# astra-vision/SceneRF

Hardware: NVIDIA H100
Metric: rays/sec (higher is better)
Workload: dtype fp32 (2 x fp16 split operands, fp32 accumulate)

## Files before the change

scenerf_b200/csrc/mlp_tc.cu:

```cuda
#include <cuda.h>
#include <cuda_fp16.h>
#include <cstdio>
#include <cstdlib>
#include <cstring>
#include <type_traits>
#include "kernels.cuh"
#include "tma.cuh"

namespace srf {
namespace tc {

constexpr int kTileM = 64;
constexpr int kChunkK = 64;
constexpr int kAChunkBytes = kTileM * 128;
constexpr int kBRows = 128, kBSlotBytes = kBRows * 128;
constexpr int kHiddenChunks = kHidden / kChunkK;
constexpr int kQuarters = kHidden / kBRows;
constexpr int kOutN = 16;
constexpr int kOutImgBytes = kOutN * 128;
constexpr int kThreads = 256;
constexpr int kNumBias = 8;
constexpr size_t kHeaderBytes = (size_t)kNumBias * kHidden * sizeof(float);
constexpr int kNumLayers = 11;
constexpr int kScaleSlot = 7 * kHidden + 256, kInvScaleSlot = 7 * kHidden + 257;
constexpr size_t kScratchFloats = (size_t)2 * kTileM * kHidden;
constexpr size_t kExchangeOffset = (size_t)2 * 2 * 64 * 128;

constexpr int kSmemAct = 0;
constexpr int kSmemX = kSmemAct + kHiddenChunks * kAChunkBytes;
constexpr int kSmemZ = kSmemX + kAChunkBytes;
constexpr int kRingBytes = 4 * kBSlotBytes;
constexpr int kSmemRing = kSmemZ + 2 * kAChunkBytes;
constexpr int kSmemBar = kSmemRing + 2 * kRingBytes;
constexpr int kSmemSph = kSmemBar + 2 * 4 * 8;
constexpr int kSmemMask = kSmemSph + kTileM * 4;
constexpr int kSmemTotal = kSmemMask + 16;
static_assert(kSmemTotal + 1024 <= 232448, "shared memory budget");

struct Layer { int chunks_is_kz, chunks, fresh, signal, is_out; };
__constant__ Layer kLayers[kNumLayers] = {
    {0, 1, 1, 0, 0}, {1, 0, 0, 1, 0},
    {0, 8, 1, 1, 0}, {0, 8, 1, 0, 0}, {1, 0, 0, 1, 0},
    {0, 8, 1, 1, 0}, {0, 8, 1, 0, 0}, {1, 0, 0, 1, 0},
    {0, 8, 1, 1, 0}, {0, 8, 1, 1, 0},
    {0, 8, 1, 1, 1}};

struct KernelArgs {
  const float* pts;
  const float* viewdir;
  int n, n_per, n_tiles, kz;
  const unsigned char* wblob;
  float* scratch;
  float* raw_out;
  int d_out;
  int32_t* dbg_sphere;
  int skip_zero;
  int hidden_fp16;
  const unsigned char* preproj;
  int pre_W1, pre_H1;
  int debug_layer;
  float* debug_acc;
  int* error_flag;
};

__device__ __forceinline__ void fence_proxy_async_smem() { asm volatile("fence.proxy.async.shared::cta;" ::: "memory"); }

__device__ __forceinline__ uint64_t l2_policy_evict_last() {
  uint64_t pol;
  asm volatile("createpolicy.fractional.L2::evict_last.b64 %0, 1.0;" : "=l"(pol));
  return pol;
}
__device__ __forceinline__ void bulk_g2s(uint32_t dst_smem, const void* src, uint32_t bytes, uint32_t bar, uint64_t policy) {
  asm volatile("cp.async.bulk.shared::cluster.global.mbarrier::complete_tx::bytes.L2::cache_hint [%0], [%1], %2, [%3], %4;"
               ::"r"(dst_smem), "l"(src), "r"(bytes), "r"(bar), "l"(policy)
               : "memory");
}
__device__ __forceinline__ void named_bar_sync(int id, int threads) {
  asm volatile("bar.sync %0, %1;" ::"r"(id), "r"(threads) : "memory");
}
__device__ __forceinline__ void sts128(uint32_t addr, uint32_t a, uint32_t b, uint32_t c, uint32_t d) {
  asm volatile("st.shared.v4.b32 [%0], {%1, %2, %3, %4};" ::"r"(addr), "r"(a), "r"(b), "r"(c), "r"(d) : "memory");
}
__device__ __forceinline__ void sts32(uint32_t addr, uint32_t a) {
  asm volatile("st.shared.b32 [%0], %1;" ::"r"(addr), "r"(a) : "memory");
}
__device__ __forceinline__ uint32_t pack_relu_half2(float lo, float hi) {
  uint32_t d;
  asm("cvt.rn.relu.f16x2.f32 %0, %1, %2;" : "=r"(d) : "f"(hi), "f"(lo));
  return d;
}
__device__ __forceinline__ uint32_t pack_half2(float lo, float hi) {
  __half2 h = __floats2half2_rn(lo, hi);
  return *reinterpret_cast<uint32_t*>(&h);
}
__device__ __forceinline__ void split_half2(float a, float b, uint32_t& hi, uint32_t& lo) {
  const __half2 h = __floats2half2_rn(a, b);
  const float2 hf = __half22float2(h);
  const __half2 l = __floats2half2_rn(a - hf.x, b - hf.y);
  hi = *reinterpret_cast<const uint32_t*>(&h);
  lo = *reinterpret_cast<const uint32_t*>(&l);
}

__device__ __forceinline__ uint32_t sw128_offset(int row, int g) { return (uint32_t)(row * 128 + ((g ^ (row & 7)) << 4)); }

__device__ __forceinline__ int layer_chunks(int l, int kz) { return kLayers[l].chunks_is_kz ? kz : kLayers[l].chunks; }
__device__ __forceinline__ bool chunk_active(int l, int c, uint64_t mask) { return !kLayers[l].chunks_is_kz || ((mask >> c) & 1ull); }

__device__ __forceinline__ uint64_t chunk_mask_for_scales(const DevParams& p, uint32_t scale_bits, int kz) {
  uint64_t m = 0;
  for (int c = 0; c < kz; ++c) {
    const int lo = c * kChunkK, hi = lo + kChunkK;
    for (int s = 0; s < kScales; ++s)
      if (((scale_bits >> s) & 1u) && p.ch_off[s] < hi && p.ch_off[s + 1] > lo) m |= 1ull << c;
  }
  return m;
}

__device__ __forceinline__ size_t chunk_image_offset(int l, int k, int kz, int parts) {
  size_t off = 0;
  for (int i = 0; i < l; ++i) off += (size_t)layer_chunks(i, kz) * (kLayers[i].is_out ? kOutImgBytes : kQuarters * kBSlotBytes);
  return (off + (size_t)k * (kLayers[l].is_out ? kOutImgBytes : kQuarters * kBSlotBytes)) * (size_t)parts;
}

struct Cursor {
  int l = 0, k = 0, j = 0;
  __device__ __forceinline__ bool normalize(int kz, uint64_t mask, int last_layer, int wg) {
    while (l <= last_layer) {
      if (l == kNumLayers - 1 && wg != 0) return false;
      if (j >= (kLayers[l].is_out ? 1 : 2)) { j = 0; ++k; }
      if (k >= layer_chunks(l, kz)) { k = 0; ++l; continue; }
      if (!chunk_active(l, k, mask)) { ++k; continue; }
      return true;
    }
    return false;
  }
};

__device__ __forceinline__ int next_active(int kz, uint64_t mask, int c) {
  for (++c; c < kz; ++c)
    if ((mask >> c) & 1ull) return c;
  return -1;
}

template <bool H16, bool SPLIT, bool PRE>
__global__ void __launch_bounds__(kThreads, 1)
point_mlp_tc_kernel(const __grid_constant__ DevParams p, const __grid_constant__ KernelArgs a) {
  extern __shared__ __align__(1024) unsigned char smem_dyn[];
  unsigned char* smem = smem_dyn + ((1024u - (smem_u32(smem_dyn) & 1023u)) & 1023u);
  const uint32_t smem_base = smem_u32(smem);
  const int tid = threadIdx.x;
  const int wg = tid >> 7, t = tid & 127, w = t >> 5, lane = tid & 31;
  constexpr int kParts = SPLIT ? 2 : 1;
  constexpr int kPts = SPLIT ? kTileM / 2 : kTileM;
  constexpr int kSlotBytes = kBSlotBytes * kParts;
  constexpr int kSlots = kRingBytes / kSlotBytes;
  const uint32_t ring = smem_base + kSmemRing + (uint32_t)wg * kRingBytes;
  auto full_bar = [&](int s) { return smem_base + kSmemBar + 8u * (uint32_t)(wg * 4 + s); };
  short2* sph_smem = reinterpret_cast<short2*>(smem + kSmemSph);
  volatile unsigned long long* mask_smem = reinterpret_cast<volatile unsigned long long*>(smem + kSmemMask);

  if (tid == 0) {
    for (int s = 0; s < 8; ++s) mbar_init(smem_base + kSmemBar + 8u * s, 1);
    fence_barrier_init();
  }
  __syncthreads();

  const int kz = a.kz;
  const int last_layer = (a.debug_layer >= 0) ? a.debug_layer : (kNumLayers - 1);
  const unsigned char* images = a.wblob + kHeaderBytes;
  const float* bias = reinterpret_cast<const float*>(a.wblob);
  float* scratch = a.scratch + (size_t)blockIdx.x * kScratchFloats;
  float* hbuf = scratch + (size_t)wg * (2 * 64 * 128);
  float* xbuf = scratch + kExchangeOffset + (size_t)wg * (2 * 64 * 64);
  const uint64_t policy = l2_policy_evict_last();

  Cursor pc;
  bool p_live = false;
  uint32_t ppos = 0, cpos = 0, done = 0;
  uint64_t mask = 0;
  auto produce = [&]() {
    if (t != 0) return;
    while (p_live && ppos < done + (uint32_t)kSlots) {
      const bool is_out = kLayers[pc.l].is_out != 0;
      const unsigned char* src = images + chunk_image_offset(pc.l, pc.k, kz, kParts) + (is_out ? 0 : (size_t)(2 * wg + pc.j) * kSlotBytes);
      const uint32_t bytes = is_out ? (uint32_t)(kOutImgBytes * kParts) : (uint32_t)kSlotBytes;
      const int s = (int)(ppos % kSlots);
      mbar_arrive_expect_tx(full_bar(s), bytes);
      bulk_g2s(ring + (uint32_t)s * kSlotBytes, src, bytes, full_bar(s), policy);
      ++ppos;
      ++pc.j;
      p_live = pc.normalize(kz, mask, last_layer, wg);
    }
  };
  float acc0[64], acc1[64], acco[8];
  auto wait_slot = [&]() -> uint32_t {
    const int s = (int)(cpos % kSlots);
    mbar_wait<kWatchPointMlp>(full_bar(s), (cpos / kSlots) & 1u, a.error_flag);
    return ring + (uint32_t)s * kSlotBytes;
  };
  auto release1 = [&]() {
    gmma::wait<1>();
    done = cpos - 1;
    produce();
  };
  auto mma_pair = [&](uint32_t a_addr, bool fresh) {
    const uint64_t ad = gmma::desc_sw128(a_addr);
    {
      const uint32_t b = wait_slot();
      gmma::fence();
#pragma unroll
      for (int k = 0; k < 4; ++k)
#pragma unroll
        for (int part = 0; part < kParts; ++part)
          gmma::mma_f16_n128(acc0, ad + 2 * k, gmma::desc_sw128(b + part * kBSlotBytes) + 2 * k, (fresh && k == 0 && part == 0) ? 0 : 1);
      gmma::commit();
      ++cpos;
    }
    release1();
    {
      const uint32_t b = wait_slot();
      gmma::fence();
#pragma unroll
      for (int k = 0; k < 4; ++k)
#pragma unroll
        for (int part = 0; part < kParts; ++part)
          gmma::mma_f16_n128(acc1, ad + 2 * k, gmma::desc_sw128(b + part * kBSlotBytes) + 2 * k, (fresh && k == 0 && part == 0) ? 0 : 1);
      gmma::commit();
      ++cpos;
    }
  };
  auto mma_out = [&](uint32_t a_addr, bool fresh) {
    const uint64_t ad = gmma::desc_sw128(a_addr);
    const uint32_t b = wait_slot();
    gmma::fence();
#pragma unroll
    for (int k = 0; k < 4; ++k)
#pragma unroll
      for (int part = 0; part < kParts; ++part)
        gmma::mma_f16_n16(acco, ad + 2 * k, gmma::desc_sw128(b + part * kOutImgBytes) + 2 * k, (fresh && k == 0 && part == 0) ? 0 : 1);
    gmma::commit();
    ++cpos;
  };
  auto retire1 = release1;
  auto retire0 = [&]() {
    gmma::wait<0>();
    gmma::fence_regs(acc0); gmma::fence_regs(acc1); gmma::fence_regs(acco);
    done = cpos;
    produce();
  };
  auto sync_all = [&]() { named_bar_sync(1, kThreads); };

  const short2* sph_cur = sph_smem;
  const int erow0 = 16 * w + (lane >> 2);
  const int ecol = 2 * (lane & 3);

  for (int tile = blockIdx.x; tile < a.n_tiles; tile += gridDim.x) {
    const int row0 = tile * kPts;
    if (tid == 0) mask_smem[0] = 0ull;
    sync_all();
    {
      uint32_t my_scales = 0;
      if (tid < kPts) {
        const int gi = row0 + tid;
        int sx = kSphereInvalid, sy = kSphereInvalid;
        if (gi < a.n) {
          point_to_sphere(p, a.pts[(size_t)gi * 3 + 0], a.pts[(size_t)gi * 3 + 1], a.pts[(size_t)gi * 3 + 2], sx, sy);
          if (a.dbg_sphere) { a.dbg_sphere[(size_t)gi * 2 + 0] = sx; a.dbg_sphere[(size_t)gi * 2 + 1] = sy; }
        }
        sph_smem[tid] = make_short2((short)max(min(sx, 32767), -32768), (short)max(min(sy, 32767), -32768));
        if (a.skip_zero) {
#pragma unroll
          for (int s = 0; s < kScales; ++s) my_scales |= scale_taps(p, s, sx, sy).any ? (1u << s) : 0u;
        }
      }
      if (a.skip_zero && tid < ((kPts + 31) & ~31)) {
        const uint32_t wbits = __reduce_or_sync(0xffffffffu, my_scales);
        if (lane == 0) {
          const unsigned long long bits = chunk_mask_for_scales(p, wbits, kz);
          if (bits) atomicOr((unsigned long long*)mask_smem, bits);
        }
      }
    }
    sync_all();
    mask = PRE ? 0ull : (a.skip_zero ? mask_smem[0] : ~0ull);
    pc = Cursor();
    p_live = pc.normalize(kz, mask, last_layer, wg);
    produce();

    const unsigned char* pre_row[2] = {nullptr, nullptr};
    if constexpr (PRE) {
#pragma unroll
      for (int hh = 0; hh < 2; ++hh) {
        const short2 sp = sph_cur[(erow0 + 8 * hh) % kPts];
        const bool in = sp.x >= 0 && sp.x < a.pre_W1 && sp.y >= 0 && sp.y < a.pre_H1;
        const size_t ridx = in ? (size_t)sp.y * a.pre_W1 + sp.x : (size_t)a.pre_W1 * a.pre_H1;
        pre_row[hh] = a.preproj + ridx * (size_t)(SRF_NUM_BLOCKS * kHidden * (SPLIT ? 4 : 2));
      }
    }

    if (tid < 2 * kPts) {
      const bool first = tid < kPts;
      const int xrow = first ? tid : tid - kPts;
      const int gi = row0 + xrow;
      const uint32_t slot_addr = smem_base + kSmemX;
      float qx = 0.f, qy = 0.f, qz = 0.f;
      if (gi < a.n) { qx = a.pts[(size_t)gi * 3 + 0]; qy = a.pts[(size_t)gi * 3 + 1]; qz = a.pts[(size_t)gi * 3 + 2]; }
      const float kPi = 3.14159274101257324f, kHalfPi = 1.57079637050628662f;
      auto sel3 = [](int i, float v0, float v1, float v2) { return i == 0 ? v0 : (i == 1 ? v1 : v2); };
      auto xval = [&](int idx, const float* vd) -> float {
        if (gi >= a.n) return 0.0f;
        if (idx < 3) return sel3(idx, qx, qy, qz);
        if (idx < 3 + 36) {
          const int j = idx - 3, fp = j / 3, cc = j - 3 * fp;
          float arg = fmul(sel3(cc, qx, qy, qz), kPi * (float)(1 << (fp >> 1)));
          if (fp & 1) arg = fadd(kHalfPi, arg);
          return sinf(arg);
        }
        if (idx < kDX) return sel3(idx - 39, vd[0], vd[1], vd[2]);
        return 0.0f;
      };
      float vd[3] = {0.f, 0.f, 0.f};
      if (!first && gi < a.n) {
        const float* vp = a.viewdir + (size_t)(gi / a.n_per) * 3;
        vd[0] = vp[0]; vd[1] = vp[1]; vd[2] = vp[2];
      }
      const int g_end = first ? 3 : 8;
#pragma unroll 1
      for (int g = first ? 0 : 3; g < g_end; ++g) {
        float v[8];
#pragma unroll
        for (int j = 0; j < 8; ++j) v[j] = xval(8 * g + j, vd);
        if constexpr (SPLIT) {
          uint32_t hi[4], lo[4];
#pragma unroll
          for (int j = 0; j < 4; ++j) split_half2(v[2 * j], v[2 * j + 1], hi[j], lo[j]);
          sts128(slot_addr + sw128_offset(xrow, g), hi[0], hi[1], hi[2], hi[3]);
          sts128(slot_addr + sw128_offset(xrow + kPts, g), lo[0], lo[1], lo[2], lo[3]);
        } else {
          sts128(slot_addr + sw128_offset(xrow, g), pack_half2(v[0], v[1]), pack_half2(v[2], v[3]), pack_half2(v[4], v[5]),
                 pack_half2(v[6], v[7]));
        }
      }
    }
    fence_proxy_async_smem();
    sync_all();

    constexpr int kItems = kPts / 32;
    int cur_scale = -1;
    int t_off[kItems];
    uint32_t t_ok[kItems];
    float t_w[kItems], t_n[kItems];
    int dxo = 0, dyo = 0;
    auto gather = [&](int c, uint32_t zaddr) {
      const int g = tid & 7;
      const int ch = c * kChunkK + g * 8;
      auto emit_vals = [&](int row, const float (&v)[8]) {
        if constexpr (SPLIT) {
          uint32_t hi[4], lo[4];
#pragma unroll
          for (int j = 0; j < 4; ++j) split_half2(v[2 * j], v[2 * j + 1], hi[j], lo[j]);
          sts128(zaddr + sw128_offset(row, g), hi[0], hi[1], hi[2], hi[3]);
          sts128(zaddr + sw128_offset(row + kPts, g), lo[0], lo[1], lo[2], lo[3]);
        } else {
          sts128(zaddr + sw128_offset(row, g), pack_half2(v[0], v[1]), pack_half2(v[2], v[3]), pack_half2(v[4], v[5]), pack_half2(v[6], v[7]));
        }
      };
      int s = -1;
#pragma unroll
      for (int i = 0; i < kScales; ++i)
        if (ch >= p.ch_off[i] && ch < p.ch_off[i + 1]) s = i;
      if (s >= 0 && s != cur_scale) {
        dxo = p.C[s]; dyo = p.W[s] * p.C[s];
#pragma unroll
        for (int i = 0; i < kItems; ++i) {
          const short2 sp16 = sph_cur[(tid >> 3) + 32 * i];
          const Taps tp = scale_taps(p, s, sp16.x, sp16.y);
          t_ok[i] = (tp.off[0] >= 0 ? 1u : 0u) | (tp.off[1] >= 0 ? 2u : 0u) | (tp.off[2] >= 0 ? 4u : 0u) | (tp.off[3] >= 0 ? 8u : 0u);
          int o0 = 0;
          if (tp.off[0] >= 0) o0 = tp.off[0];
          else if (tp.off[1] >= 0) o0 = tp.off[1] - dxo;
          else if (tp.off[2] >= 0) o0 = tp.off[2] - dyo;
          else if (tp.off[3] >= 0) o0 = tp.off[3] - dxo - dyo;
          t_off[i] = o0;
          t_w[i] = tp.fx; t_n[i] = tp.fy;
        }
        cur_scale = s;
      }
      const char* fbytes = (s >= 0) ? reinterpret_cast<const char*>(p.feat[s]) : nullptr;
      const int ch_in = (s >= 0) ? ch - p.ch_off[s] : 0;
      const bool f16 = p.feat_fp16 != 0;
#pragma unroll
      for (int u = 0; u < kItems; ++u) {
        const int row = (tid >> 3) + 32 * u;
        float acc[8];
        const uint32_t ok = (s >= 0) ? t_ok[u] : 0u;
        if (!ok) {
#pragma unroll
          for (int e = 0; e < 8; ++e) acc[e] = 0.0f;
          emit_vals(row, acc);
          continue;
        }
        const float wx = t_w[u], ny = t_n[u];
        const float e_ = fsub(1.0f, wx), so = fsub(1.0f, ny);
        const float tw4[4] = {fmul(so, e_), fmul(so, wx), fmul(ny, e_), fmul(ny, wx)};
        float v[4][8];
#pragma unroll
        for (int tp = 0; tp < 4; ++tp) {
          if ((ok >> tp) & 1u) {
            const size_t eidx = (size_t)(ch_in + t_off[u] + (tp & 1) * dxo + (tp >> 1) * dyo);
            if (f16) {
              const uint4 raw = __ldg(reinterpret_cast<const uint4*>(fbytes + eidx * 2));
              const uint32_t rw[4] = {raw.x, raw.y, raw.z, raw.w};
#pragma unroll
              for (int q = 0; q < 4; ++q) {
                const float2 f = __half22float2(*reinterpret_cast<const __half2*>(&rw[q]));
                v[tp][2 * q] = f.x; v[tp][2 * q + 1] = f.y;
              }
            } else {
              const float4* src = reinterpret_cast<const float4*>(fbytes + eidx * 4);
              const float4 a0 = __ldg(src), a1 = __ldg(src + 1);
              v[tp][0] = a0.x; v[tp][1] = a0.y; v[tp][2] = a0.z; v[tp][3] = a0.w;
              v[tp][4] = a1.x; v[tp][5] = a1.y; v[tp][6] = a1.z; v[tp][7] = a1.w;
            }
          } else {
#pragma unroll
            for (int e = 0; e < 8; ++e) v[tp][e] = 0.0f;
          }
        }
#pragma unroll
        for (int e = 0; e < 8; ++e) {
          acc[e] = fmul(v[0][e], tw4[0]);
#pragma unroll
          for (int tp = 1; tp < 4; ++tp) acc[e] = fadd(acc[e], fmul(v[tp][e], tw4[tp]));
        }
        emit_vals(row, acc);
      }
    };
    auto zpass = [&]() {
      cur_scale = -1;
      int c = next_active(kz, mask, -1);
      if (c < 0) return;
      gather(c, smem_base + kSmemZ);
      fence_proxy_async_smem();
      sync_all();
      for (int zi = 0; c >= 0; ++zi) {
        const int cn = next_active(kz, mask, c);
        mma_pair(smem_base + kSmemZ + (uint32_t)(zi & 1) * kAChunkBytes, false);
        if (cn >= 0) gather(cn, smem_base + kSmemZ + (uint32_t)((zi + 1) & 1) * kAChunkBytes);
        retire0();
        fence_proxy_async_smem();
        sync_all();
        c = cn;
      }
    };

    auto epilogue = [&](auto use_h_c, auto write_h_c, auto use_p_c, int bias_idx) __attribute__((always_inline)) {
      constexpr bool USE_H = decltype(use_h_c)::value, WRITE_H = decltype(write_h_c)::value, USE_P = decltype(use_p_c)::value;
      [[maybe_unused]] const float inv_scale = SPLIT ? __ldg(bias + kInvScaleSlot) : 1.0f;
      [[maybe_unused]] float* xs = reinterpret_cast<float*>(smem + kSmemZ + (size_t)wg * kAChunkBytes);
      auto finish = [&](float (&acc)[64], int j) __attribute__((always_inline)) {
#pragma unroll
       for (int half = 0; half < 2; ++half) {
        if constexpr (SPLIT) {
          if (j | half) named_bar_sync(2 + wg, 128);
          if (t >= 64) {
#pragma unroll
            for (int i = 0; i < 32; ++i) xs[i * 64 + (t - 64)] = acc[32 * half + i];
          }
          named_bar_sync(2 + wg, 128);
          if (t >= 64) continue;
        }
#pragma unroll
        for (int i2 = 16 * half; i2 < 16 * half + 16; ++i2) {
          const int i = 2 * i2, hh = i2 & 1;
          const int row = erow0 + 8 * hh;
          const int col = 256 * wg + 128 * j + 8 * (i2 >> 1) + ecol;
          float r0 = acc[i], r1 = acc[i + 1];
          if constexpr (SPLIT) {
            const float p0 = xs[(i - 32 * half) * 64 + t], p1 = xs[(i + 1 - 32 * half) * 64 + t];
            r0 = (r0 + p0) * inv_scale; r1 = (r1 + p1) * inv_scale;
          }
          if constexpr (!USE_P) {
            const float2 bb = __ldg(reinterpret_cast<const float2*>(bias + (size_t)bias_idx * kHidden + col));
            r0 += bb.x; r1 += bb.y;
          }
          [[maybe_unused]] float2* hp = reinterpret_cast<float2*>(hbuf) + (size_t)(j * 32 + i2) * 128 + t;
          [[maybe_unused]] __half2* hp16 = reinterpret_cast<__half2*>(hbuf) + (size_t)(j * 32 + i2) * 128 + t;
          if constexpr (USE_H) {
            if constexpr (H16) { const float2 f = __half22float2(*hp16); r0 += f.x; r1 += f.y; }
            else { const float2 f = *hp; r0 += f.x; r1 += f.y; }
          }
          if constexpr (USE_P) {
            if constexpr (SPLIT) {
              const float2 f = __ldg(reinterpret_cast<const float2*>(pre_row[hh] + ((size_t)bias_idx * kHidden + col) * 4));
              r0 += f.x; r1 += f.y;
            } else {
              const float2 f = __half22float2(__ldg(reinterpret_cast<const __half2*>(pre_row[hh] + ((size_t)bias_idx * kHidden + col) * 2)));
              r0 += f.x; r1 += f.y;
            }
          }
          if constexpr (WRITE_H) {
            if constexpr (H16) *hp16 = __floats2half2_rn(r0, r1);
            else *hp = make_float2(r0, r1);
          }
          const uint32_t addr = smem_base + kSmemAct + (uint32_t)(col >> 6) * kAChunkBytes;
          const uint32_t inrow = (uint32_t)((((col & 63) >> 3) ^ (row & 7)) << 4) + (uint32_t)((col & 7) * 2);
          if constexpr (SPLIT) {
            uint32_t hi, lo;
            split_half2(fmaxf(r0, 0.0f), fmaxf(r1, 0.0f), hi, lo);
            sts32(addr + (uint32_t)row * 128 + inrow, hi);
            sts32(addr + (uint32_t)(row + kPts) * 128 + inrow, lo);
          } else {
            sts32(addr + (uint32_t)row * 128 + inrow, pack_relu_half2(r0, r1));
          }
        }
       }
      };
      finish(acc0, 0);
      finish(acc1, 1);
    };
    auto epi = [&](auto use_h_c, auto write_h_c, auto use_p_c, int bias_idx) __attribute__((always_inline)) {
      retire0();
      sync_all();
      epilogue(use_h_c, write_h_c, use_p_c, bias_idx);
      fence_proxy_async_smem();
      sync_all();
    };
    auto dump_acc = [&](bool out) {
      retire0();
      if (out && wg != 0) return;
#pragma unroll
      for (int hh = 0; hh < 2; ++hh) {
        float* dst = a.debug_acc + ((size_t)tile * kTileM + erow0 + 8 * hh) * kHidden;
        if (out) {
#pragma unroll
          for (int c8 = 0; c8 < 2; ++c8) { dst[8 * c8 + ecol] = acco[4 * c8 + 2 * hh]; dst[8 * c8 + ecol + 1] = acco[4 * c8 + 2 * hh + 1]; }
        } else {
#pragma unroll
          for (int c8 = 0; c8 < 16; ++c8) {
            const int col = 256 * wg + 8 * c8 + ecol;
            dst[col] = acc0[4 * c8 + 2 * hh]; dst[col + 1] = acc0[4 * c8 + 2 * hh + 1];
            dst[col + 128] = acc1[4 * c8 + 2 * hh]; dst[col + 129] = acc1[4 * c8 + 2 * hh + 1];
          }
        }
      }
    };

    using T = std::true_type;
    using F = std::false_type;
    using P = std::integral_constant<bool, PRE>;
    mma_pair(smem_base + kSmemX, true);
    retire1();
    if (!PRE) zpass();
    if (a.debug_layer == 1) { dump_acc(false); continue; }
    bool stop = false;
    for (int b = 0; b < SRF_NUM_BLOCKS; ++b) {
      if (b == 0) epi(F{}, T{}, P{}, b);
      else epi(T{}, T{}, P{}, b);
#pragma unroll 1
      for (int k = 0; k < kHiddenChunks; ++k) { mma_pair(smem_base + kSmemAct + (uint32_t)k * kAChunkBytes, k == 0); retire1(); }
      if (a.debug_layer == 2 + 3 * b) { dump_acc(false); stop = true; break; }
      epi(F{}, F{}, F{}, 3 + b);
#pragma unroll 1
      for (int k = 0; k < kHiddenChunks; ++k) { mma_pair(smem_base + kSmemAct + (uint32_t)k * kAChunkBytes, k == 0); retire1(); }
      if (b < SRF_NUM_BLOCKS - 1) {
        if (!PRE) zpass();
        if (a.debug_layer == 4 + 3 * b) { dump_acc(false); stop = true; break; }
      } else if (a.debug_layer == 9) { dump_acc(false); stop = true; break; }
    }
    if (stop) continue;
    epi(T{}, F{}, F{}, 6);
    if (wg == 0) {
#pragma unroll 1
      for (int k = 0; k < kHiddenChunks; ++k) { mma_out(smem_base + kSmemAct + (uint32_t)k * kAChunkBytes, k == 0); retire1(); }
      if (a.debug_layer == 10) { dump_acc(true); continue; }
      retire0();
      const float* bo = bias + (size_t)7 * kHidden;
      if constexpr (SPLIT) {
        if (t >= 64) {
#pragma unroll
          for (int i = 0; i < 8; ++i) xbuf[i * 64 + (t - 64)] = acco[i];
        }
        named_bar_sync(2, 128);
      }
      if (!SPLIT || t < 64) {
        const float inv_scale = SPLIT ? __ldg(bias + kInvScaleSlot) : 1.0f;
#pragma unroll
        for (int i = 0; i < 8; ++i) {
          const int row = erow0 + 8 * ((i >> 1) & 1);
          const int col = 8 * (i >> 2) + ecol + (i & 1);
          float v = acco[i];
          if constexpr (SPLIT) v = (v + xbuf[i * 64 + t]) * inv_scale;
          const int gi = row0 + row;
          if (row < kPts && gi < a.n && col < a.d_out) a.raw_out[(size_t)gi * a.d_out + col] = v + __ldg(bo + col);
        }
      }
    }
  }
}

struct PackArgs {
  srf_mlp_weights w;
  int kz;
  int parts;
};

__device__ __forceinline__ const float* layer_weight(const srf_mlp_weights& w, int l, int& K) {
  K = kHidden;
  switch (l) {
    case 0: K = kDX; return w.lin_in_w;
    case 1: K = w.d_latent; return w.lin_z_w[0];
    case 2: return w.fc0_w[0];
    case 3: return w.fc1_w[0];
    case 4: K = w.d_latent; return w.lin_z_w[1];
    case 5: return w.fc0_w[1];
    case 6: return w.fc1_w[1];
    case 7: K = w.d_latent; return w.lin_z_w[2];
    case 8: return w.fc0_w[2];
    case 9: return w.fc1_w[2];
    default: return w.lin_out_w;
  }
}

__global__ void weight_absmax_kernel(const __grid_constant__ PackArgs pa, unsigned int* __restrict__ max_bits) {
  float m = 0.0f;
  for (int l = 0; l < kNumLayers; ++l) {
    int K;
    const float* W = layer_weight(pa.w, l, K);
    const size_t n = (size_t)(l == kNumLayers - 1 ? pa.w.d_out : kHidden) * K;
    for (size_t i = (size_t)blockIdx.x * blockDim.x + threadIdx.x; i < n; i += (size_t)gridDim.x * blockDim.x) m = fmaxf(m, fabsf(W[i]));
  }
#pragma unroll
  for (int o = 16; o > 0; o >>= 1) m = fmaxf(m, __shfl_xor_sync(0xffffffffu, m, o));
  if ((threadIdx.x & 31) == 0) atomicMax(max_bits, __float_as_uint(m));
}
__global__ void weight_scale_kernel(const unsigned int* __restrict__ max_bits, float* __restrict__ hdr, int split) {
  float scale = 1.0f;
  if (split) {
    const float m = __uint_as_float(*max_bits);
    int e = 0;
    if (m > 0.0f && isfinite(m)) { frexpf(m, &e); e = 14 - e; }
    e = max(-40, min(40, e));
    scale = ldexpf(1.0f, e);
  }
  hdr[kScaleSlot] = scale;
  hdr[kInvScaleSlot] = 1.0f / scale;
}

__global__ void pack_images_kernel(const __grid_constant__ PackArgs pa, const float* __restrict__ hdr, unsigned char* __restrict__ images,
                                   size_t n_granules) {
  const size_t gid = (size_t)blockIdx.x * blockDim.x + threadIdx.x;
  if (gid >= n_granules) return;
  size_t byte = gid * 16;
  const int parts = pa.parts;
  const float scale = hdr[kScaleSlot];
  int l = 0;
  size_t off = 0;
  for (; l < kNumLayers; ++l) {
    const size_t sz = (size_t)layer_chunks(l, pa.kz) * (kLayers[l].is_out ? kOutImgBytes : kQuarters * kBSlotBytes) * parts;
    if (byte < off + sz) break;
    off += sz;
  }
  const size_t rel = byte - off;
  const bool is_out = kLayers[l].is_out;
  const size_t img_bytes = is_out ? kOutImgBytes : kBSlotBytes;
  const size_t chunk_bytes = (is_out ? 1 : kQuarters) * img_bytes * parts;
  const int c = (int)(rel / chunk_bytes);
  const size_t in_chunk = rel % chunk_bytes;
  const int img = (int)(in_chunk / img_bytes);
  const int q = img / parts, part = img % parts;
  const size_t in_img = in_chunk % img_bytes;
  const int row = (int)(in_img / 128);
  const int gpos = (int)((in_img % 128) / 16);
  const int g = gpos ^ (row & 7);
  const int n = q * kBRows + row;
  int K;
  const float* W = layer_weight(pa.w, l, K);
  const int n_rows = is_out ? pa.w.d_out : kHidden;
  __align__(16) __half hv[8];
#pragma unroll
  for (int j = 0; j < 8; ++j) {
    const int k = c * kChunkK + g * 8 + j;
    const float v = ((n < n_rows && k < K) ? W[(size_t)n * K + k] : 0.0f) * scale;
    const __half hi = __float2half_rn(v);
    hv[j] = part == 0 ? hi : __float2half_rn(v - __half2float(hi));
  }
  *reinterpret_cast<uint4*>(images + byte) = *reinterpret_cast<const uint4*>(hv);
}

__global__ void pack_header_kernel(const __grid_constant__ PackArgs pa, float* __restrict__ hdr) {
  const int j = blockIdx.x * blockDim.x + threadIdx.x;
  if (j >= kHidden) return;
  const srf_mlp_weights& w = pa.w;
  hdr[0 * kHidden + j] = w.lin_in_b[j] + w.lin_z_b[0][j];
  hdr[1 * kHidden + j] = w.fc1_b[0][j] + w.lin_z_b[1][j];
  hdr[2 * kHidden + j] = w.fc1_b[1][j] + w.lin_z_b[2][j];
  hdr[3 * kHidden + j] = w.fc0_b[0][j];
  hdr[4 * kHidden + j] = w.fc0_b[1][j];
  hdr[5 * kHidden + j] = w.fc0_b[2][j];
  hdr[6 * kHidden + j] = w.fc1_b[2][j];
  hdr[7 * kHidden + j] = (j < w.d_out) ? w.lin_out_b[j] : 0.0f;
}

static size_t images_bytes(int kz, int parts = 1) {
  size_t b = 0;
  const int chunks[kNumLayers] = {1, kz, 8, 8, kz, 8, 8, kz, 8, 8, 8};
  for (int l = 0; l < kNumLayers; ++l) b += (size_t)chunks[l] * (l == kNumLayers - 1 ? kOutImgBytes : kQuarters * kBSlotBytes);
  return b * (size_t)parts;
}

}

static inline int kz_of(int d_latent) { return (d_latent + tc::kChunkK - 1) / tc::kChunkK; }

size_t tc_weights_bytes(int d_out, int d_latent, int split) {
  (void)d_out;
  return tc::kHeaderBytes + tc::images_bytes(kz_of(d_latent), split ? 2 : 1) + 256;
}

int pack_weights_tc(const srf_mlp_weights& w, void* dst, size_t bytes, int split, cudaStream_t st) {
  const int kz = kz_of(w.d_latent);
  if (kz > 64 || w.d_out < 1 || w.d_out > tc::kOutN || (w.d_latent % 8)) return 1;
  const size_t need = tc_weights_bytes(w.d_out, w.d_latent, split);
  if (bytes < need) return 1;
  tc::PackArgs pa;
  pa.w = w;
  pa.kz = kz;
  pa.parts = split ? 2 : 1;
  float* hdr = reinterpret_cast<float*>(dst);
  unsigned int* max_bits = reinterpret_cast<unsigned int*>(reinterpret_cast<unsigned char*>(dst) + need - 4);
  tc::pack_header_kernel<<<(kHidden + 127) / 128, 128, 0, st>>>(pa, hdr);
  if (split) {
    cudaMemsetAsync(max_bits, 0, 4, st);
    tc::weight_absmax_kernel<<<296, 256, 0, st>>>(pa, max_bits);
  }
  tc::weight_scale_kernel<<<1, 1, 0, st>>>(max_bits, hdr, split ? 1 : 0);
  const size_t n_gran = tc::images_bytes(kz, pa.parts) / 16;
  tc::pack_images_kernel<<<(unsigned)((n_gran + 255) / 256), 256, 0, st>>>(
      pa, hdr, reinterpret_cast<unsigned char*>(dst) + tc::kHeaderBytes, n_gran);
  return 0;
}

static int num_sms() { return device_sm_count(); }

using TcKernelFn = void (*)(const DevParams, const tc::KernelArgs);
constexpr int kNumTcKernels = 6;
static TcKernelFn tc_kernel_at(int i) {
  static const TcKernelFn table[kNumTcKernels] = {
      tc::point_mlp_tc_kernel<false, false, false>, tc::point_mlp_tc_kernel<true, false, false>, tc::point_mlp_tc_kernel<false, true, false>,
      tc::point_mlp_tc_kernel<false, false, true>,  tc::point_mlp_tc_kernel<true, false, true>,  tc::point_mlp_tc_kernel<false, true, true>};
  return table[i];
}
static TcKernelFn tc_kernel(bool h16, bool split, bool pre) { return tc_kernel_at((split ? 2 : (h16 ? 1 : 0)) + (pre ? 3 : 0)); }

constexpr int kMaxTcCtas = 256;
size_t tc_workspace_bytes(int d_latent, int n_points) {
  (void)d_latent; (void)n_points;
  return (size_t)kMaxTcCtas * tc::kScratchFloats * sizeof(float) + 256;
}

int run_point_mlp_tc_debug(const DevParams& p, const srf_mlp_weights& w, const float* pts, const float* viewdir, int n,
                           int n_per, float* raw_out, int32_t* dbg_sphere, int flags, void* workspace, size_t ws_bytes,
                           int debug_layer, float* debug_acc, cudaStream_t st) {
  if (ws_bytes < tc_workspace_bytes(p.d_latent, n)) return -1;
  if (debug_layer >= 0 && !(debug_layer < tc::kNumLayers && debug_layer != 0 && debug_layer != 3 && debug_layer != 6))
    return -2;
  const size_t smem = tc::kSmemTotal + 1024;
  static bool attr_set = false;
  if (!attr_set) {
    for (int i = 0; i < kNumTcKernels; ++i) cudaFuncSetAttribute(tc_kernel_at(i), cudaFuncAttributeMaxDynamicSharedMemorySize, (int)smem);
    attr_set = true;
  }
  const bool split = (flags & kTcFlagSplit) != 0;
  const int tile_pts = split ? tc::kTileM / 2 : tc::kTileM;
  tc::KernelArgs a;
  a.pts = pts; a.viewdir = viewdir; a.n = n; a.n_per = n_per;
  a.n_tiles = (n + tile_pts - 1) / tile_pts;
  a.kz = kz_of(p.d_latent);
  a.wblob = reinterpret_cast<const unsigned char*>(split ? w.tc_split_packed : w.tc_packed);
  if (!a.wblob) return -3;
  a.scratch = reinterpret_cast<float*>(workspace);
  a.raw_out = raw_out; a.d_out = w.d_out; a.dbg_sphere = dbg_sphere;
  a.skip_zero = (flags & SRF_FLAG_SKIP_ZERO_CHUNKS) ? 1 : 0;
  a.hidden_fp16 = (!split && (flags & SRF_FLAG_HIDDEN_FP16)) ? 1 : 0;
  a.preproj = nullptr; a.pre_W1 = p.sphere_W + 1; a.pre_H1 = p.sphere_H + 1;
  if ((flags & kTcFlagPreproj) && p.preproj && (p.preproj_fp16 != 0) == !split) {
    a.preproj = reinterpret_cast<const unsigned char*>(p.preproj);
    a.skip_zero = 0;
  }
  a.debug_layer = debug_layer; a.debug_acc = debug_acc;
  a.error_flag = watchdog_device_flag();
  int grid = a.n_tiles < num_sms() ? a.n_tiles : num_sms();
  if (grid > kMaxTcCtas) grid = kMaxTcCtas;
  if (grid < 1) return 0;
  tc_kernel(a.hidden_fp16 != 0, split, a.preproj != nullptr)<<<grid, tc::kThreads, smem, st>>>(p, a);
  return 1;
}

int run_point_mlp_tc(const DevParams& p, const srf_mlp_weights& w, const float* pts, const float* viewdir, int n,
                     int n_per, float* raw_out, int32_t* dbg_sphere, int flags, void* workspace, size_t ws_bytes,
                     cudaStream_t st) {
  return run_point_mlp_tc_debug(p, w, pts, viewdir, n, n_per, raw_out, dbg_sphere, flags, workspace, ws_bytes, -1,
                                nullptr, st);
}

}
```

Measured before the change: 64800.

## Split A operand into hi/lo activations so split mode uses full 64-row tiles

Split-precision mode now stores both fp16 hi and lo parts of activations in shared memory and issues two MMAs per B slice against the same weight image, instead of splitting the weight into two parts and processing only 32 points per tile. This doubles points per tile and removes the cross-thread exchange of partial accumulators through scratch. To fit registers, hidden layers flush half-K partial sums to global scratch mid-layer and add them back in the epilogue. The shared memory layout is made template-dependent, with the split path using a 3-slot ring and reusing the activation space for the X and Z buffers. This adds extra global scratch traffic and a mid-layer flush, and the B-operand packing must now match the new per-slot indexing.

```diff
diff --git a/scenerf_b200/csrc/mlp_tc.cu b/scenerf_b200/csrc/mlp_tc.cu
--- a/scenerf_b200/csrc/mlp_tc.cu
+++ b/scenerf_b200/csrc/mlp_tc.cu
@@ -24,18 +24,27 @@
 constexpr int kNumLayers = 11;
 constexpr int kScaleSlot = 7 * kHidden + 256, kInvScaleSlot = 7 * kHidden + 257;
 constexpr size_t kScratchFloats = (size_t)2 * kTileM * kHidden;
-constexpr size_t kExchangeOffset = (size_t)2 * 2 * 64 * 128;
-
-constexpr int kSmemAct = 0;
-constexpr int kSmemX = kSmemAct + kHiddenChunks * kAChunkBytes;
-constexpr int kSmemZ = kSmemX + kAChunkBytes;
-constexpr int kRingBytes = 4 * kBSlotBytes;
-constexpr int kSmemRing = kSmemZ + 2 * kAChunkBytes;
-constexpr int kSmemBar = kSmemRing + 2 * kRingBytes;
-constexpr int kSmemSph = kSmemBar + 2 * 4 * 8;
-constexpr int kSmemMask = kSmemSph + kTileM * 4;
-constexpr int kSmemTotal = kSmemMask + 16;
-static_assert(kSmemTotal + 1024 <= 232448, "shared memory budget");
+
+template <bool SPLIT>
+struct Smem {
+  static constexpr int kParts = SPLIT ? 2 : 1;
+  static constexpr int kAStride = kParts * kAChunkBytes;
+  static constexpr int kAct = 0;
+  static constexpr int kX = SPLIT ? kAct : kAct + kHiddenChunks * kAStride;
+  static constexpr int kZ = SPLIT ? kAct + kAStride : kX + kAStride;
+  static constexpr int kSlots = SPLIT ? 3 : 4;
+  static constexpr int kRingBytes = kSlots * kBSlotBytes;
+  static constexpr int kRing = SPLIT ? kAct + kHiddenChunks * kAStride : kZ + 2 * kAStride;
+  static constexpr int kBar = kRing + 2 * kRingBytes;
+  static constexpr int kSph = kBar + 2 * 4 * 8;
+  static constexpr int kMask = kSph + kTileM * 4;
+  static constexpr int kTotal = kMask + 16;
+};
+static_assert(Smem<false>::kRing == 88 * 1024 && Smem<false>::kTotal + 1024 <= 232448, "shared memory budget (fp16)");
+using SmemSplit = Smem<true>;
+static_assert(SmemSplit::kRing == 128 * 1024 && SmemSplit::kTotal + 1024 <= 232448, "shared memory budget (split)");
+static_assert(SmemSplit::kZ >= SmemSplit::kX + SmemSplit::kAStride &&
+              SmemSplit::kZ + 2 * SmemSplit::kAStride <= SmemSplit::kAct + 7 * SmemSplit::kAStride, "split latent buffers");
 
 struct Layer { int chunks_is_kz, chunks, fresh, signal, is_out; };
 __constant__ Layer kLayers[kNumLayers] = {
@@ -122,12 +131,13 @@
   return (off + (size_t)k * (kLayers[l].is_out ? kOutImgBytes : kQuarters * kBSlotBytes)) * (size_t)parts;
 }
 
+template <int kWideSlots>
 struct Cursor {
   int l = 0, k = 0, j = 0;
   __device__ __forceinline__ bool normalize(int kz, uint64_t mask, int last_layer, int wg) {
     while (l <= last_layer) {
       if (l == kNumLayers - 1 && wg != 0) return false;
-      if (j >= (kLayers[l].is_out ? 1 : 2)) { j = 0; ++k; }
+      if (j >= (kLayers[l].is_out ? 1 : kWideSlots)) { j = 0; ++k; }
       if (k >= layer_chunks(l, kz)) { k = 0; ++l; continue; }
       if (!chunk_active(l, k, mask)) { ++k; continue; }
       return true;
@@ -150,17 +160,20 @@
   const uint32_t smem_base = smem_u32(smem);
   const int tid = threadIdx.x;
   const int wg = tid >> 7, t = tid & 127, w = t >> 5, lane = tid & 31;
-  constexpr int kParts = SPLIT ? 2 : 1;
-  constexpr int kPts = SPLIT ? kTileM / 2 : kTileM;
-  constexpr int kSlotBytes = kBSlotBytes * kParts;
-  constexpr int kSlots = kRingBytes / kSlotBytes;
-  const uint32_t ring = smem_base + kSmemRing + (uint32_t)wg * kRingBytes;
-  auto full_bar = [&](int s) { return smem_base + kSmemBar + 8u * (uint32_t)(wg * 4 + s); };
-  short2* sph_smem = reinterpret_cast<short2*>(smem + kSmemSph);
-  volatile unsigned long long* mask_smem = reinterpret_cast<volatile unsigned long long*>(smem + kSmemMask);
+  using L = Smem<SPLIT>;
+  constexpr int kParts = L::kParts;
+  constexpr int kPts = kTileM;
+  constexpr int kWideSlots = 2 * kParts;
+  constexpr int kSlots = L::kSlots;
+  constexpr int kAStride = L::kAStride;
+  constexpr int kSmemAct = L::kAct, kSmemX = L::kX, kSmemZ = L::kZ;
+  const uint32_t ring = smem_base + L::kRing + (uint32_t)wg * L::kRingBytes;
+  auto full_bar = [&](int s) { return smem_base + L::kBar + 8u * (uint32_t)(wg * 4 + s); };
+  short2* sph_smem = reinterpret_cast<short2*>(smem + L::kSph);
+  volatile unsigned long long* mask_smem = reinterpret_cast<volatile unsigned long long*>(smem + L::kMask);
 
   if (tid == 0) {
-    for (int s = 0; s < 8; ++s) mbar_init(smem_base + kSmemBar + 8u * s, 1);
+    for (int s = 0; s < 8; ++s) mbar_init(smem_base + L::kBar + 8u * s, 1);
     fence_barrier_init();
   }
   __syncthreads();
@@ -171,10 +184,10 @@
   const float* bias = reinterpret_cast<const float*>(a.wblob);
   float* scratch = a.scratch + (size_t)blockIdx.x * kScratchFloats;
   float* hbuf = scratch + (size_t)wg * (2 * 64 * 128);
-  float* xbuf = scratch + kExchangeOffset + (size_t)wg * (2 * 64 * 64);
+  [[maybe_unused]] float* pbuf = scratch + (size_t)(2 + wg) * (2 * 64 * 128);
   const uint64_t policy = l2_policy_evict_last();
 
-  Cursor pc;
+  Cursor<kWideSlots> pc;
   bool p_live = false;
   uint32_t ppos = 0, cpos = 0, done = 0;
   uint64_t mask = 0;
@@ -182,11 +195,11 @@
     if (t != 0) return;
     while (p_live && ppos < done + (uint32_t)kSlots) {
       const bool is_out = kLayers[pc.l].is_out != 0;
-      const unsigned char* src = images + chunk_image_offset(pc.l, pc.k, kz, kParts) + (is_out ? 0 : (size_t)(2 * wg + pc.j) * kSlotBytes);
-      const uint32_t bytes = is_out ? (uint32_t)(kOutImgBytes * kParts) : (uint32_t)kSlotBytes;
+      const unsigned char* src = images + chunk_image_offset(pc.l, pc.k, kz, kParts) + (is_out ? 0 : (size_t)(kWideSlots * wg + pc.j) * kBSlotBytes);
+      const uint32_t bytes = is_out ? (uint32_t)(kOutImgBytes * kParts) : (uint32_t)kBSlotBytes;
       const int s = (int)(ppos % kSlots);
       mbar_arrive_expect_tx(full_bar(s), bytes);
-      bulk_g2s(ring + (uint32_t)s * kSlotBytes, src, bytes, full_bar(s), policy);
+      bulk_g2s(ring + (uint32_t)s * kBSlotBytes, src, bytes, full_bar(s), policy);
       ++ppos;
       ++pc.j;
       p_live = pc.normalize(kz, mask, last_layer, wg);
@@ -196,48 +209,68 @@
   auto wait_slot = [&]() -> uint32_t {
     const int s = (int)(cpos % kSlots);
     mbar_wait<kWatchPointMlp>(full_bar(s), (cpos / kSlots) & 1u, a.error_flag);
-    return ring + (uint32_t)s * kSlotBytes;
+    return ring + (uint32_t)s * kBSlotBytes;
   };
   auto release1 = [&]() {
     gmma::wait<1>();
     done = cpos - 1;
     produce();
   };
+  auto mma_image = [&](float (&acc)[64], uint64_t ad_hi, uint64_t ad_lo, bool fresh) __attribute__((always_inline)) {
+    const uint64_t bd = gmma::desc_sw128(wait_slot());
+    gmma::fence();
+#pragma unroll
+    for (int k = 0; k < 4; ++k) {
+      gmma::mma_f16_n128(acc, ad_hi + 2 * k, bd + 2 * k, (fresh && k == 0) ? 0 : 1);
+      gmma::mma_f16_n128(acc, ad_lo + 2 * k, bd + 2 * k, 1);
+    }
+    gmma::commit();
+    ++cpos;
+  };
   auto mma_pair = [&](uint32_t a_addr, bool fresh) {
     const uint64_t ad = gmma::desc_sw128(a_addr);
-    {
-      const uint32_t b = wait_slot();
-      gmma::fence();
-#pragma unroll
-      for (int k = 0; k < 4; ++k)
-#pragma unroll
-        for (int part = 0; part < kParts; ++part)
-          gmma::mma_f16_n128(acc0, ad + 2 * k, gmma::desc_sw128(b + part * kBSlotBytes) + 2 * k, (fresh && k == 0 && part == 0) ? 0 : 1);
-      gmma::commit();
-      ++cpos;
-    }
-    release1();
-    {
-      const uint32_t b = wait_slot();
-      gmma::fence();
-#pragma unroll
-      for (int k = 0; k < 4; ++k)
-#pragma unroll
-        for (int part = 0; part < kParts; ++part)
-          gmma::mma_f16_n128(acc1, ad + 2 * k, gmma::desc_sw128(b + part * kBSlotBytes) + 2 * k, (fresh && k == 0 && part == 0) ? 0 : 1);
-      gmma::commit();
-      ++cpos;
+    if constexpr (SPLIT) {
+      const uint64_t ad_lo = gmma::desc_sw128(a_addr + kAChunkBytes);
+      mma_image(acc0, ad, ad_lo, fresh);
+      release1();
+      mma_image(acc0, ad, ad_lo, false);
+      release1();
+      mma_image(acc1, ad, ad_lo, fresh);
+      release1();
+      mma_image(acc1, ad, ad_lo, false);
+    } else {
+      {
+        const uint32_t b = wait_slot();
+        gmma::fence();
+#pragma unroll
+        for (int k = 0; k < 4; ++k) gmma::mma_f16_n128(acc0, ad + 2 * k, gmma::desc_sw128(b) + 2 * k, (fresh && k == 0) ? 0 : 1);
+        gmma::commit();
+        ++cpos;
+      }
+      release1();
+      {
+        const uint32_t b = wait_slot();
+        gmma::fence();
+#pragma unroll
+        for (int k = 0; k < 4; ++k) gmma::mma_f16_n128(acc1, ad + 2 * k, gmma::desc_sw128(b) + 2 * k, (fresh && k == 0) ? 0 : 1);
+        gmma::commit();
+        ++cpos;
+      }
     }
   };
   auto mma_out = [&](uint32_t a_addr, bool fresh) {
     const uint64_t ad = gmma::desc_sw128(a_addr);
+    [[maybe_unused]] const uint64_t ad_lo = gmma::desc_sw128(a_addr + kAChunkBytes);
     const uint32_t b = wait_slot();
     gmma::fence();
 #pragma unroll
     for (int k = 0; k < 4; ++k)
 #pragma unroll
-      for (int part = 0; part < kParts; ++part)
-        gmma::mma_f16_n16(acco, ad + 2 * k, gmma::desc_sw128(b + part * kOutImgBytes) + 2 * k, (fresh && k == 0 && part == 0) ? 0 : 1);
+      for (int part = 0; part < kParts; ++part) {
+        const uint64_t bd = gmma::desc_sw128(b + part * kOutImgBytes) + 2 * k;
+        gmma::mma_f16_n16(acco, ad + 2 * k, bd, (fresh && k == 0 && part == 0) ? 0 : 1);
+        if constexpr (SPLIT) gmma::mma_f16_n16(acco, ad_lo + 2 * k, bd, 1);
+      }
     gmma::commit();
     ++cpos;
   };
@@ -249,6 +282,16 @@
     produce();
   };
   auto sync_all = [&]() { named_bar_sync(1, kThreads); };
+  auto flush = [&]() {
+    retire0();
+#pragma unroll
+    for (int i2 = 0; i2 < 32; ++i2) {
+      reinterpret_cast<float2*>(pbuf)[(size_t)i2 * 128 + t] = make_float2(acc0[2 * i2], acc0[2 * i2 + 1]);
+      reinterpret_cast<float2*>(pbuf)[(size_t)(32 + i2) * 128 + t] = make_float2(acc1[2 * i2], acc1[2 * i2 + 1]);
+    }
+#pragma unroll
+    for (int i = 0; i < 64; ++i) { acc0[i] = 0.0f; acc1[i] = 0.0f; }
+  };
 
   const short2* sph_cur = sph_smem;
   const int erow0 = 16 * w + (lane >> 2);
@@ -283,7 +326,7 @@
     }
     sync_all();
     mask = PRE ? 0ull : (a.skip_zero ? mask_smem[0] : ~0ull);
-    pc = Cursor();
+    pc = Cursor<kWideSlots>();
     p_live = pc.normalize(kz, mask, last_layer, wg);
     produce();
 
@@ -440,13 +483,14 @@
       cur_scale = -1;
       int c = next_active(kz, mask, -1);
       if (c < 0) return;
+      if constexpr (SPLIT) sync_all();
       gather(c, smem_base + kSmemZ);
       fence_proxy_async_smem();
       sync_all();
       for (int zi = 0; c >= 0; ++zi) {
         const int cn = next_active(kz, mask, c);
-        mma_pair(smem_base + kSmemZ + (uint32_t)(zi & 1) * kAChunkBytes, false);
-        if (cn >= 0) gather(cn, smem_base + kSmemZ + (uint32_t)((zi + 1) & 1) * kAChunkBytes);
+        mma_pair(smem_base + kSmemZ + (uint32_t)(zi & 1) * kAStride, false);
+        if (cn >= 0) gather(cn, smem_base + kSmemZ + (uint32_t)((zi + 1) & 1) * kAStride);
         retire0();
         fence_proxy_async_smem();
         sync_all();
@@ -456,30 +500,22 @@
 
     auto epilogue = [&](auto use_h_c, auto write_h_c, auto use_p_c, int bias_idx) __attribute__((always_inline)) {
       constexpr bool USE_H = decltype(use_h_c)::value, WRITE_H = decltype(write_h_c)::value, USE_P = decltype(use_p_c)::value;
+      constexpr bool PART = SPLIT && (USE_H || !WRITE_H);
       [[maybe_unused]] const float inv_scale = SPLIT ? __ldg(bias + kInvScaleSlot) : 1.0f;
-      [[maybe_unused]] float* xs = reinterpret_cast<float*>(smem + kSmemZ + (size_t)wg * kAChunkBytes);
+      int erow = erow0;
+      if constexpr (SPLIT) asm volatile("mov.b32 %0, %0;" : "+r"(erow));
       auto finish = [&](float (&acc)[64], int j) __attribute__((always_inline)) {
 #pragma unroll
-       for (int half = 0; half < 2; ++half) {
-        if constexpr (SPLIT) {
-          if (j | half) named_bar_sync(2 + wg, 128);
-          if (t >= 64) {
-#pragma unroll
-            for (int i = 0; i < 32; ++i) xs[i * 64 + (t - 64)] = acc[32 * half + i];
-          }
-          named_bar_sync(2 + wg, 128);
-          if (t >= 64) continue;
-        }
-#pragma unroll
-        for (int i2 = 16 * half; i2 < 16 * half + 16; ++i2) {
+        for (int i2 = 0; i2 < 32; ++i2) {
           const int i = 2 * i2, hh = i2 & 1;
-          const int row = erow0 + 8 * hh;
+          const int row = erow + 8 * hh;
           const int col = 256 * wg + 128 * j + 8 * (i2 >> 1) + ecol;
           float r0 = acc[i], r1 = acc[i + 1];
-          if constexpr (SPLIT) {
-            const float p0 = xs[(i - 32 * half) * 64 + t], p1 = xs[(i + 1 - 32 * half) * 64 + t];
-            r0 = (r0 + p0) * inv_scale; r1 = (r1 + p1) * inv_scale;
+          if constexpr (PART) {
+            const float2 f = reinterpret_cast<const float2*>(pbuf)[(size_t)(j * 32 + i2) * 128 + t];
+            r0 += f.x; r1 += f.y;
           }
+          if constexpr (SPLIT) { r0 *= inv_scale; r1 *= inv_scale; }
           if constexpr (!USE_P) {
             const float2 bb = __ldg(reinterpret_cast<const float2*>(bias + (size_t)bias_idx * kHidden + col));
             r0 += bb.x; r1 += bb.y;
@@ -503,7 +539,7 @@
             if constexpr (H16) *hp16 = __floats2half2_rn(r0, r1);
             else *hp = make_float2(r0, r1);
           }
-          const uint32_t addr = smem_base + kSmemAct + (uint32_t)(col >> 6) * kAChunkBytes;
+          const uint32_t addr = smem_base + kSmemAct + (uint32_t)(col >> 6) * kAStride;
           const uint32_t inrow = (uint32_t)((((col & 63) >> 3) ^ (row & 7)) << 4) + (uint32_t)((col & 7) * 2);
           if constexpr (SPLIT) {
             uint32_t hi, lo;
@@ -514,7 +550,6 @@
             sts32(addr + (uint32_t)row * 128 + inrow, pack_relu_half2(r0, r1));
           }
         }
-       }
       };
       finish(acc0, 0);
       finish(acc1, 1);
@@ -526,12 +561,19 @@
       fence_proxy_async_smem();
       sync_all();
     };
-    auto dump_acc = [&](bool out) {
+    auto dump_acc = [&](bool out, bool part) {
       retire0();
       if (out && wg != 0) return;
 #pragma unroll
       for (int hh = 0; hh < 2; ++hh) {
-        float* dst = a.debug_acc + ((size_t)tile * kTileM + erow0 + 8 * hh) * kHidden;
+        float* dst;
+        if constexpr (SPLIT) {
+          const int gi = row0 + erow0 + 8 * hh;
+          if (gi >= a.n) continue;
+          dst = a.debug_acc + ((size_t)(gi >> 5) * 64 + (gi & 31)) * kHidden;
+        } else {
+          dst = a.debug_acc + ((size_t)tile * kTileM + erow0 + 8 * hh) * kHidden;
+        }
         if (out) {
 #pragma unroll
           for (int c8 = 0; c8 < 2; ++c8) { dst[8 * c8 + ecol] = acco[4 * c8 + 2 * hh]; dst[8 * c8 + ecol + 1] = acco[4 * c8 + 2 * hh + 1]; }
@@ -539,8 +581,17 @@
 #pragma unroll
           for (int c8 = 0; c8 < 16; ++c8) {
             const int col = 256 * wg + 8 * c8 + ecol;
-            dst[col] = acc0[4 * c8 + 2 * hh]; dst[col + 1] = acc0[4 * c8 + 2 * hh + 1];
-            dst[col + 128] = acc1[4 * c8 + 2 * hh]; dst[col + 129] = acc1[4 * c8 + 2 * hh + 1];
+            float v[4] = {acc0[4 * c8 + 2 * hh], acc0[4 * c8 + 2 * hh + 1], acc1[4 * c8 + 2 * hh], acc1[4 * c8 + 2 * hh + 1]};
+            if constexpr (SPLIT) {
+              if (part) {
+                const int i2 = 2 * c8 + hh;
+                const float2 p0 = reinterpret_cast<const float2*>(pbuf)[(size_t)i2 * 128 + t];
+                const float2 p1 = reinterpret_cast<const float2*>(pbuf)[(size_t)(32 + i2) * 128 + t];
+                v[0] += p0.x; v[1] += p0.y; v[2] += p1.x; v[3] += p1.y;
+              }
+            }
+            dst[col] = v[0]; dst[col + 1] = v[1];
+            dst[col + 128] = v[2]; dst[col + 129] = v[3];
           }
         }
       }
@@ -552,48 +603,47 @@
     mma_pair(smem_base + kSmemX, true);
     retire1();
     if (!PRE) zpass();
-    if (a.debug_layer == 1) { dump_acc(false); continue; }
+    if (a.debug_layer == 1) { dump_acc(false, false); continue; }
     bool stop = false;
     for (int b = 0; b < SRF_NUM_BLOCKS; ++b) {
       if (b == 0) epi(F{}, T{}, P{}, b);
       else epi(T{}, T{}, P{}, b);
 #pragma unroll 1
-      for (int k = 0; k < kHiddenChunks; ++k) { mma_pair(smem_base + kSmemAct + (uint32_t)k * kAChunkBytes, k == 0); retire1(); }
-      if (a.debug_layer == 2 + 3 * b) { dump_acc(false); stop = true; break; }
+      for (int k = 0; k < kHiddenChunks; ++k) {
+        mma_pair(smem_base + kSmemAct + (uint32_t)k * kAStride, k == 0);
+        retire1();
+        if (SPLIT && k == kHiddenChunks / 2 - 1) flush();
+      }
+      if (a.debug_layer == 2 + 3 * b) { dump_acc(false, true); stop = true; break; }
       epi(F{}, F{}, F{}, 3 + b);
 #pragma unroll 1
-      for (int k = 0; k < kHiddenChunks; ++k) { mma_pair(smem_base + kSmemAct + (uint32_t)k * kAChunkBytes, k == 0); retire1(); }
+      for (int k = 0; k < kHiddenChunks; ++k) {
+        mma_pair(smem_base + kSmemAct + (uint32_t)k * kAStride, k == 0);
+        retire1();
+        if (SPLIT && k == kHiddenChunks / 2 - 1) flush();
+      }
       if (b < SRF_NUM_BLOCKS - 1) {
         if (!PRE) zpass();
-        if (a.debug_layer == 4 + 3 * b) { dump_acc(false); stop = true; break; }
-      } else if (a.debug_layer == 9) { dump_acc(false); stop = true; break; }
+        if (a.debug_layer == 4 + 3 * b) { dump_acc(false, true); stop = true; break; }
+      } else if (a.debug_layer == 9) { dump_acc(false, true); stop = true; break; }
     }
     if (stop) continue;
     epi(T{}, F{}, F{}, 6);
     if (wg == 0) {
 #pragma unroll 1
-      for (int k = 0; k < kHiddenChunks; ++k) { mma_out(smem_base + kSmemAct + (uint32_t)k * kAChunkBytes, k == 0); retire1(); }
-      if (a.debug_layer == 10) { dump_acc(true); continue; }
+      for (int k = 0; k < kHiddenChunks; ++k) { mma_out(smem_base + kSmemAct + (uint32_t)k * kAStride, k == 0); retire1(); }
+      if (a.debug_layer == 10) { dump_acc(true, false); continue; }
       retire0();
       const float* bo = bias + (size_t)7 * kHidden;
-      if constexpr (SPLIT) {
-        if (t >= 64) {
-#pragma unroll
-          for (int i = 0; i < 8; ++i) xbuf[i * 64 + (t - 64)] = acco[i];
-        }
-        named_bar_sync(2, 128);
-      }
-      if (!SPLIT || t < 64) {
-        const float inv_scale = SPLIT ? __ldg(bias + kInvScaleSlot) : 1.0f;
-#pragma unroll
-        for (int i = 0; i < 8; ++i) {
-          const int row = erow0 + 8 * ((i >> 1) & 1);
-          const int col = 8 * (i >> 2) + ecol + (i & 1);
-          float v = acco[i];
-          if constexpr (SPLIT) v = (v + xbuf[i * 64 + t]) * inv_scale;
-          const int gi = row0 + row;
-          if (row < kPts && gi < a.n && col < a.d_out) a.raw_out[(size_t)gi * a.d_out + col] = v + __ldg(bo + col);
-        }
+      const float inv_scale = SPLIT ? __ldg(bias + kInvScaleSlot) : 1.0f;
+#pragma unroll
+      for (int i = 0; i < 8; ++i) {
+        const int row = erow0 + 8 * ((i >> 1) & 1);
+        const int col = 8 * (i >> 2) + ecol + (i & 1);
+        float v = acco[i];
+        if constexpr (SPLIT) v *= inv_scale;
+        const int gi = row0 + row;
+        if (gi < a.n && col < a.d_out) a.raw_out[(size_t)gi * a.d_out + col] = v + __ldg(bo + col);
       }
     }
   }
@@ -765,17 +815,18 @@
   if (ws_bytes < tc_workspace_bytes(p.d_latent, n)) return -1;
   if (debug_layer >= 0 && !(debug_layer < tc::kNumLayers && debug_layer != 0 && debug_layer != 3 && debug_layer != 6))
     return -2;
-  const size_t smem = tc::kSmemTotal + 1024;
+  const bool split = (flags & kTcFlagSplit) != 0;
+  auto smem_of = [](bool s) { return (size_t)(s ? tc::Smem<true>::kTotal : tc::Smem<false>::kTotal) + 1024; };
+  const size_t smem = smem_of(split);
   static bool attr_set = false;
   if (!attr_set) {
-    for (int i = 0; i < kNumTcKernels; ++i) cudaFuncSetAttribute(tc_kernel_at(i), cudaFuncAttributeMaxDynamicSharedMemorySize, (int)smem);
+    for (int i = 0; i < kNumTcKernels; ++i)
+      cudaFuncSetAttribute(tc_kernel_at(i), cudaFuncAttributeMaxDynamicSharedMemorySize, (int)smem_of(i % 3 == 2));
     attr_set = true;
   }
-  const bool split = (flags & kTcFlagSplit) != 0;
-  const int tile_pts = split ? tc::kTileM / 2 : tc::kTileM;
   tc::KernelArgs a;
   a.pts = pts; a.viewdir = viewdir; a.n = n; a.n_per = n_per;
-  a.n_tiles = (n + tile_pts - 1) / tile_pts;
+  a.n_tiles = (n + tc::kTileM - 1) / tc::kTileM;
   a.kz = kz_of(p.d_latent);
   a.wblob = reinterpret_cast<const unsigned char*>(split ? w.tc_split_packed : w.tc_packed);
   if (!a.wblob) return -3;
```

Result: faster. 75910 (median of 6 runs) (+17.1%).
